# sehyun03/MulActSeg

Measured on AMD Instinct MI355X. Metric: superpixels scored/sec, higher is better.
Workload: dtype f32

## Files before the change

### include/mulactseg_hip.h

```cpp
#ifndef MULACTSEG_HIP_H
#define MULACTSEG_HIP_H

#include <stddef.h>
#include <stdint.h>

#ifdef __cplusplus
extern "C" {
#endif

#define MAS_ID_I64 0
#define MAS_ID_I32 1
#define MAS_ID_U16 2
#define MAS_MAP_U8 3

#define MAS_MAX_CLASSES 32

#define MAS_SCORE_FRAC_BITS 40
#define MAS_PROB_FRAC_BITS 23
#define MAS_LOSS_FRAC_BITS 32

#define MAS_ABI_VERSION 9
int mas_abi_version(void);
const char* mas_error_string(int code);

// ... 50 lines not shown
                                uint64_t* gmax , uint64_t* acc , void* stream);
int mas_partial_loss_bwd_lowres(const float* zq, int h, int w, const void* spx, int spx_dtype, const uint8_t* mask,
                                const uint32_t* bits, const uint64_t* gmax, const float* scale , int N, int C, int H, int W,
                                int S, float invT, int flags, int64_t* dzq_fix , void* stream);
#define MAS_GRAD_FRAC_BITS 44
int mas_fix_to_float(const int64_t* fix, int64_t n, int frac_bits, float* out, void* stream);

size_t mas_partial_loss_work_bytes(int N, int S, int C, int flags);
int mas_partial_loss_fwd_fused(const float* z, int h, int w, const void* spx, int spx_dtype, const uint8_t* mask, const uint8_t* targets,
                               int cols_stored, int cols_used, const uint32_t* bits, int N, int C, int H, int W, int S, float invT, int flags,
                               const float* weights, void* work, size_t work_bytes, float* losses, void* stream);
int mas_partial_loss_bwd_fused(const float* z, int h, int w, const void* spx, int spx_dtype, const uint8_t* mask, const uint32_t* bits,
                               const void* work, const float* grad, const float* weights, int N, int C, int H, int W, int S, float invT,
                               int flags, float* dz, int64_t* dzq_fix, void* stream);


int mas_region_keys(const float* score, const uint8_t* valid, const int32_t* img_rank, int64_t n_img, int S,
                    uint64_t* keys , void* stream);

size_t mas_select_workspace_bytes(int64_t n);

int mas_sort_keys_desc(const uint64_t* keys_in, int64_t n, uint64_t* keys_out, void* workspace, size_t ws_bytes,
                       void* stream);

int mas_budget_walk(const uint64_t* sorted_keys, int64_t n, const uint8_t* region_cost, const int32_t* img_of_rank,
                    int S, int64_t budget, int64_t max_out, int64_t* n_selected,
                    int32_t* sel_img, int32_t* sel_id, float* sel_score, void* workspace, size_t ws_bytes, void* stream);

int mas_region_reweight(float* score, const int32_t* dominant, int64_t n, int ban_class, const float* cls_w ,
                        void* stream);

int mas_dominant_hist(const int32_t* dominant, int64_t n, int C, uint64_t* counts , void* stream);

int mas_minmax_normalize(float* scores, int64_t n, uint32_t* scratch2, void* stream);


#define MAS_LABELS_BAD_VALUE 1

int mas_region_label_counts(const void* spx, int spx_dtype, const uint8_t* labels, int H, int W, int nseg, int num_classes, int trim_k,
                            int32_t* full , int32_t* trimmed , int32_t* status ,
                            void* stream);

int mas_region_multi_hot(const int32_t* full, const int32_t* trimmed, const uint8_t* listed, int nseg, int num_classes,
                         uint8_t* bits , int64_t* size , void* stream);

int mas_region_dominant(const int32_t* full, const uint8_t* listed, const int32_t* drawn , int nseg, int num_classes,
// ... 181 lines not shown
```

### mulactseg_amd/_lib.py

```python
import ctypes
import os

_HERE = os.path.dirname(os.path.abspath(__file__))
LIB_PATH = os.environ.get("MAS_LIB") or os.path.join(_HERE, "libmulactseg_hip.so")

ID_I64, ID_I32, ID_U16 = 0, 1, 2
MAP_U8 = 3
MAX_CLASSES = 32
LABELS_BAD_VALUE = 1
SCORE_FRAC, PROB_FRAC, LOSS_FRAC = 40, 23, 32
LOSS_CE, LOSS_GROUP, LOSS_GROUP_ONLY_MULTI, LOSS_DECOMP, LOSS_TCE = 1, 2, 4, 8, 16
ACC_WORDS = 8
GRAD_FRAC = 44
MS_MAX_SOURCES = 16

SK_DMA, SK_NOSPLIT = 1, 2
LOWRES_GENERIC = 1
ABI_VERSION = 9

_c = ctypes
_vp, _i, _f, _i64, _d = _c.c_void_p, _c.c_int, _c.c_float, _c.c_int64, _c.c_double


class SkOpts(ctypes.Structure):
    _fields_ = [("flags", _c.c_uint), ("spin_limit", _c.c_uint), ("stamps", _c.c_void_p)]


SIGNATURES = {
    "mas_abi_version": (_i, []),
    "mas_error_string": (_c.c_char_p, [_i]),
    "mas_class_prob_sum": (_i, [_vp, _i, _i, _i, _i, _f, _vp, _vp]),
    "mas_bvsb_region_accum": (_i, [_vp, _vp, _i, _vp, _i, _i, _i, _i, _i, _f, _vp, _vp, _vp]),
    "mas_region_finalize": (_i, [_vp, _vp, _i64, _i, _i, _vp, _vp, _vp, _vp, _vp]),
    "mas_region_keys": (_i, [_vp, _vp, _vp, _i64, _i, _vp, _vp]),
    "mas_select_workspace_bytes": (_c.c_size_t, [_i64]),
    "mas_sort_keys_desc": (_i, [_vp, _i64, _vp, _vp, _c.c_size_t, _vp]),
    "mas_budget_walk": (_i, [_vp, _i64, _vp, _vp, _i, _i64, _i64, _vp, _vp, _vp, _vp, _vp, _c.c_size_t, _vp]),
    "mas_region_reweight": (_i, [_vp, _vp, _i64, _i, _vp, _vp]),
    "mas_dominant_hist": (_i, [_vp, _i64, _i, _vp, _vp]),
    "mas_minmax_normalize": (_i, [_vp, _i64, _vp, _vp]),
    "mas_region_label_counts": (_i, [_vp, _i, _vp, _i, _i, _i, _i, _i, _vp, _vp, _vp, _vp]),
    "mas_region_multi_hot": (_i, [_vp, _vp, _vp, _i, _i, _vp, _vp, _vp]),
    "mas_region_dominant": (_i, [_vp, _vp, _vp, _i, _i, _i, _vp, _vp]),
    "mas_region_paint": (_i, [_vp, _i, _vp, _i, _i, _i, _vp, _i, _vp, _vp]),
    "mas_spx_max_onehot": (_i, [_vp, _i, _vp, _i, _i, _i, _i, _i, _vp, _vp, _vp, _vp, _vp]),
    "mas_iou_counts": (_i, [_vp, _vp, _vp, _i64, _i, _i64, _vp, _vp]),
    "mas_logits_iou_counts": (_i, [_vp, _vp, _i, _i, _i, _i, _i, _i64, _vp, _vp]),
    "mas_single_pass_accum": (_i, [_vp, _vp, _i, _i, _i, _i, _i, _i, _f, _vp, _vp, _vp, _vp]),
    "mas_single_pass_accum_lowres": (_i, [_vp, _i, _i, _vp, _i, _i, _i, _i, _i, _i, _f, _vp, _vp, _vp, _vp]),
    "mas_single_pass_accum_lowres_opt": (_i, [_vp, _i, _i, _vp, _i, _i, _i, _i, _i, _i, _f, _vp, _vp, _vp, _c.c_uint, _vp]),
    "mas_class_weight": (_i, [_vp, _i, _i, _i64, _i, _i, _d, _vp, _vp, _vp, _vp]),
    "mas_region_finalize_weighted": (_i, [_vp, _vp, _i64, _i, _vp, _i, _vp, _vp, _vp, _vp, _vp]),
    "mas_stage2_gather_protos": (_i, [_vp, _i, _i, _i, _i, _i, _vp, _i, _vp, _vp]),
    "mas_stage2_assign": (_i, [_vp, _i, _i, _i, _i, _i, _vp, _vp, _i, _vp, _vp, _vp, _vp, _vp]),
    "mas_stage2_adjacency": (_i, [_vp, _i, _i, _i, _vp, _vp, _vp]),
    "mas_stage2_propagate": (_i, [_vp, _i, _i, _i, _i, _i, _vp, _i, _vp, _vp, _vp, _vp, _vp, _vp, _vp, _vp]),
    "mas_aspp_dw3_fwd": (_i, [_vp, _vp, _vp, _vp, _i, _i, _i, _i, _i, _i, _i, _vp, _vp, _vp, _vp]),
    "mas_aspp_dw3_bwd_x": (_i, [_vp, _vp, _vp, _vp, _vp, _vp, _i, _i, _i, _i, _i, _i, _i, _vp, _vp]),
    "mas_aspp_dw3_bwd_w": (_i, [_vp, _vp, _vp, _vp, _i, _i, _i, _i, _i, _i, _i, _vp, _vp, _vp, _vp]),
# ... 128 lines not shown
```

### mulactseg_amd/active_selection/engine.py

```python
import numpy as np
import torch


class ShardPlan:

    def __init__(self, n_img, batch_size, rank=0, world=1):
        self.n_img, self.batch_size, self.rank, self.world = n_img, batch_size, rank, world
        self.n_batches = (n_img + batch_size - 1) // batch_size
        per = (self.n_batches + world - 1) // world
        self.batch_lo = min(rank * per, self.n_batches)
        self.batch_hi = min((rank + 1) * per, self.n_batches)
        self.img_lo = min(self.batch_lo * batch_size, n_img)
        self.img_hi = min(self.batch_hi * batch_size, n_img)
        self.per_rank_imgs = per * batch_size
        self.batch_of = (np.arange(n_img) // batch_size).astype(np.int32)

    @property
    def local_indices(self):
        return list(range(self.img_lo, self.img_hi))

    @property
    def n_local(self):
        return self.img_hi - self.img_lo

# ... 68 lines not shown
    def class_weight(self, prob_sum, hw, batch_size, n_batches, coeff):
        cum, w, w31 = self.ops.class_weight(prob_sum.contiguous(), hw, batch_size, n_batches, coeff)
        w._mas_w31 = w31
        return cum, w

    def finalize_weighted(self, class_sum, hist, cls_w, ban_class, want_hist_i64=False):
        w31 = None if cls_w is None else getattr(cls_w, '_mas_w31', None)
        if w31 is None:
            w = torch.ones(hist.shape[-1], dtype=torch.float32, device=hist.device) if cls_w is None else cls_w.detach().to(hist.device)
            w31 = (w.double() * 2147483648.0).floor().to(torch.int64).view(torch.int32)[::2].contiguous()
        return self.ops.region_finalize_weighted(class_sum, hist, w31, ban_class, want_hist_i64)

    def minmax_normalize_(self, scores):
        return self.ops.minmax_normalize_(scores)

    def region_reweight_(self, scores, dominant, ban_class, cls_w):
        return self.ops.region_reweight_(scores, dominant, ban_class, cls_w)

    def dominant_hist(self, dominant, C):
        return self.ops.dominant_hist(dominant, C)

    def select(self, scores, valid, img_rank, img_of_rank, region_cost, budget, max_out):
        keys = self.ops.region_keys(scores, valid, img_rank)
        skeys = self.ops.sort_keys_desc(keys)
        nsel, simg, sid, ssc = self.ops.budget_walk(skeys, region_cost, img_of_rank, scores.shape[1], budget, max_out)
        n = int(nsel.item())
        return n, simg[:n].cpu().numpy(), sid[:n].cpu().numpy(), ssc[:n].cpu().numpy()

    def local_head(self, plan, scores, valid, img_rank, max_out):
        lo, hi = plan.img_lo, plan.img_hi
        head = torch.zeros(max_out, dtype=torch.int64, device=scores.device)
        if hi > lo:
            keys = self.ops.region_keys(scores[lo:hi].contiguous(), None if valid is None else valid[lo:hi].contiguous(),
                                        img_rank[lo:hi].contiguous())
            m = min(keys.numel(), max_out)
            head[:m] = self.ops.sort_keys_desc(keys)[:m]
        return head

    def walk_heads(self, heads, region_cost, img_of_rank, S, budget, max_out):
        nsel, simg, sid, ssc = self.ops.budget_walk(self.ops.sort_keys_desc(heads), region_cost, img_of_rank, S, budget, max_out)
        n = int(nsel.item())
        return n, simg[:n].cpu().numpy(), sid[:n].cpu().numpy(), ssc[:n].cpu().numpy()

    def select_sharded(self, plan, scores, valid, img_rank, img_of_rank, region_cost, budget, max_out):
        head = self.local_head(plan, scores, valid, img_rank, max_out)
        merged = torch.empty(plan.world * max_out, dtype=torch.int64, device=scores.device)
        _dist().all_gather_into_tensor(merged, head)
        return self.walk_heads(merged, region_cost, img_of_rank, scores.shape[1], budget, max_out)


def default_backend(device):
    return HipBackend(device)


def select_regions(backend, plan, scores, valid, img_rank, img_of_rank, region_cost, budget, max_out):
    if plan.world > 1 and max_out is not None and _dist() is not None and hasattr(backend, 'select_sharded'):
        return backend.select_sharded(plan, scores, valid, img_rank, img_of_rank, region_cost, budget, max_out)
    return backend.select(scores, valid, img_rank, img_of_rank, region_cost, budget, max_out)


class AcquisitionRound:

    def __init__(self, n_img, n_channels, n_superpixels, batch_size, temperature, backend, rank=None, world=None,
                 single_pass=False):
        r, w = current_rank_world()
# ... 97 lines not shown
```

### mulactseg_amd/csrc/select.hip

```cpp
#include <cstring>

#include <rocprim/device/device_radix_sort.hpp>
#include <rocprim/device/device_scan.hpp>

#include "common.h"

namespace {

constexpr int kThreads = 256;

__device__ __forceinline__ unsigned order_bits(float f) {
    const unsigned b = mas_f2u(f);
    return (b & 0x80000000u) ? ~b : (b | 0x80000000u);
}
__device__ __forceinline__ float unorder_bits(unsigned o) {
    return mas_u2f((o & 0x80000000u) ? (o & 0x7fffffffu) : ~o);
}

inline int id_bits_for(int S) {
    int b = 1;
    while ((1LL << b) < S) ++b;
    return b;
}

// ... 102 lines not shown
    }
#pragma unroll
    for (int off = MAS_WAVE / 2; off > 0; off >>= 1) {
        const unsigned l2 = __shfl_down(lo, off, MAS_WAVE), h2 = __shfl_down(hi, off, MAS_WAVE);
        lo = l2 < lo ? l2 : lo;
        hi = h2 > hi ? h2 : hi;
    }
    if ((threadIdx.x & (MAS_WAVE - 1)) == 0) {
        atomicMin(&mm[0], lo);
        atomicMax(&mm[1], hi);
    }
}

__global__ void k_minmax_init(unsigned* mm) { mm[0] = 0xffffffffu; mm[1] = 0u; }

__global__ __launch_bounds__(kThreads) void k_minmax_apply(float* __restrict__ u, long long n, const unsigned* __restrict__ mm) {
    const long long i = (long long)blockIdx.x * kThreads + threadIdx.x;
    if (i >= n) return;
    const float mn = unorder_bits(mm[0]);
    const float mx = unorder_bits(mm[1]) - mn;
    u[i] = (u[i] - mn) / mx;
}

inline size_t align_up(size_t v) { return (v + 255) & ~(size_t)255; }

size_t sort_temp_bytes(long long n) {
    size_t bytes = 0;
    mas_u64* nul = nullptr;
    (void)rocprim::radix_sort_keys_desc(nullptr, bytes, nul, nul, (size_t)n, 0, 64, (hipStream_t)0);
    return bytes;
}
size_t scan_temp_bytes(long long n) {
    size_t bytes = 0;
    unsigned* nul = nullptr;
    (void)rocprim::inclusive_scan(nullptr, bytes, nul, nul, (size_t)n, rocprim::plus<unsigned>(), (hipStream_t)0);
    return bytes;
}

}

extern "C" size_t mas_select_workspace_bytes(int64_t n) {
    if (n <= 0) return 0;
    const size_t t = sort_temp_bytes(n), u = scan_temp_bytes(n);
    return align_up(t > u ? t : u) + 2 * align_up(sizeof(unsigned) * (size_t)n) + 256;
}

extern "C" int mas_region_keys(const float* score, const uint8_t* valid, const int32_t* img_rank, int64_t n_img, int S,
                               uint64_t* keys, void* stream) {
    if (!score || !img_rank || !keys) return MAS_ERR_NULL;
    if (n_img <= 0 || S <= 0) return MAS_ERR_SHAPE;
    const int b = id_bits_for(S);
    if (b > 24 || n_img > (1LL << (32 - b))) return MAS_ERR_RANGE;
    const long long n = (long long)n_img * S;
    const long long nblk = (n + kThreads - 1) / kThreads;
    if (nblk > 0x7fffffffLL) return MAS_ERR_SHAPE;
    hipLaunchKernelGGL(k_region_keys, dim3((unsigned)nblk), dim3(kThreads), 0, static_cast<hipStream_t>(stream), score, valid,
                       img_rank, n, S, b, reinterpret_cast<mas_u64*>(keys));
    return mas_launch_status();
}

extern "C" int mas_sort_keys_desc(const uint64_t* keys_in, int64_t n, uint64_t* keys_out, void* workspace, size_t ws_bytes,
                                  void* stream) {
    if (!keys_in || !keys_out || !workspace) return MAS_ERR_NULL;
    if (n <= 0) return MAS_ERR_SHAPE;
    size_t need = sort_temp_bytes(n);
    if (ws_bytes < need) return MAS_ERR_WORKSPACE;
    hipError_t e = rocprim::radix_sort_keys_desc(workspace, need, reinterpret_cast<const mas_u64*>(keys_in),
                                                 reinterpret_cast<mas_u64*>(keys_out), (size_t)n, 0, 64,
                                                 static_cast<hipStream_t>(stream));
    return e == hipSuccess ? mas_launch_status() : (int)e;
}

extern "C" int mas_budget_walk(const uint64_t* sorted_keys, int64_t n, const uint8_t* region_cost, const int32_t* img_of_rank,
                               int S, int64_t budget, int64_t max_out, int64_t* n_selected, int32_t* sel_img, int32_t* sel_id,
                               float* sel_score, void* workspace, size_t ws_bytes, void* stream) {
    if (!sorted_keys || !img_of_rank || !n_selected || !sel_img || !sel_id || !sel_score || !workspace) return MAS_ERR_NULL;
    if (n <= 0 || S <= 0 || max_out <= 0 || budget < 0) return MAS_ERR_SHAPE;
    if (n > (1LL << 24)) return MAS_ERR_RANGE;
    if (ws_bytes < mas_select_workspace_bytes(n)) return MAS_ERR_WORKSPACE;
    hipStream_t st = static_cast<hipStream_t>(stream);
    const int b = id_bits_for(S);
    unsigned char* ws = static_cast<unsigned char*>(workspace);
    size_t temp = scan_temp_bytes(n);
    const size_t t = sort_temp_bytes(n);
    const size_t temp_region = align_up(t > temp ? t : temp);
    unsigned* cost = reinterpret_cast<unsigned*>(ws + temp_region);
    unsigned* prefix = reinterpret_cast<unsigned*>(ws + temp_region + align_up(sizeof(unsigned) * (size_t)n));
    const mas_u64* keys = reinterpret_cast<const mas_u64*>(sorted_keys);
    unsigned long long* nsel = reinterpret_cast<unsigned long long*>(n_selected);
    const long long nblk = (n + kThreads - 1) / kThreads;
    hipLaunchKernelGGL(k_set_u64, dim3(1), dim3(1), 0, st, nsel, (unsigned long long)n);
    hipLaunchKernelGGL(k_walk_cost, dim3((unsigned)nblk), dim3(kThreads), 0, st, keys, (long long)n, region_cost, img_of_rank, S, b, cost);
// ... 41 lines not shown
```

### mulactseg_amd/csrc/single_pass.hip

```cpp
#include <cstdlib>
#include "common.h"

namespace {

constexpr int kThreads = 256;
constexpr int kTileW = 256;
constexpr int kTileH = 16;
constexpr int kLogSlots = 7;
constexpr int kSlots = 1 << kLogSlots;

__device__ __forceinline__ int table_slot(int* keys, int id) {
    unsigned h = ((unsigned)id * 2654435769u) >> (32 - kLogSlots);
    for (int probe = 0; probe < kSlots; ++probe) {
        int k = __hip_atomic_load(&keys[h], __ATOMIC_RELAXED, __HIP_MEMORY_SCOPE_WORKGROUP);
        if (k == id) return (int)h;
        if (k == -1) {
            int old = atomicCAS(&keys[h], -1, id);
            if (old == -1 || old == id) return (int)h;
        }
        h = (h + 1) & (kSlots - 1);
    }
    return -1;
}

// ... 284 lines not shown
    __device__ __forceinline__ void load(const unsigned short* p) { a = *reinterpret_cast<const uint2*>(p); }
    __device__ __forceinline__ void get(int (&id)[4]) const {
        id[0] = (int)(a.x & 0xffffu); id[1] = (int)(a.x >> 16); id[2] = (int)(a.y & 0xffffu); id[3] = (int)(a.y >> 16);
    }
};

template <int CT, typename IdT>
struct RowRegs {
    float4 t[CT];
    IdQuad<IdT> ids;
};

template <int CT, bool EXACT, typename IdT>
__device__ __forceinline__ void ring_issue(RowRegs<CT, IdT>& r, const float* __restrict__ zb, const IdT* __restrict__ sb, int C,
                                           int HW, unsigned off) {
    r.ids.load(sb + off);
#pragma unroll
    for (int c = 0; c < CT; ++c) {
        if (EXACT || c < C) r.t[c] = mas_load_stream4(zb + (size_t)c * HW + off);
        else r.t[c] = make_float4(0.f, 0.f, 0.f, 0.f);
    }
}

template <int CT, bool EXACT, typename IdT>
__device__ __forceinline__ void ring_consume(RowRegs<CT, IdT>& r, bool ok, int C, int S, float invT, unsigned* s_acc, int* t_keys,
                                             mas_u64* t_sum, unsigned* t_hist, mas_u64* __restrict__ gsum,
                                             unsigned* __restrict__ ghist, int& last_id, int& last_slot) {
    mas_v2f v[2][CT];
    float b1[4], b2[4];
    int a1[4];
#pragma unroll
    for (int k = 0; k < 4; ++k) { b1[k] = -__builtin_inff(); b2[k] = -__builtin_inff(); a1[k] = 0; }
#pragma unroll
    for (int c = 0; c < CT; ++c) {
        if (EXACT || c < C) {
            const float4 t = r.t[c];
            v[0][c] = (mas_v2f){t.x, t.y};
            v[1][c] = (mas_v2f){t.z, t.w};
            const float q[4] = {t.x, t.y, t.z, t.w};
#pragma unroll
            for (int k = 0; k < 4; ++k) {
                const bool g1 = q[k] > b1[k];
                b2[k] = __builtin_amdgcn_fmed3f(b1[k], b2[k], q[k]);
                a1[k] = g1 ? c : a1[k];
                b1[k] = __builtin_amdgcn_fmed3f(b1[k], q[k], 3.402823466e+38f);
            }
        } else {
            v[0][c] = mas_splat(0.f);
            v[1][c] = mas_splat(0.f);
        }
    }
    __builtin_amdgcn_sched_barrier(0);
    {
        mas_v2f Ra, Rb;
        mas_softmax_quad<CT, EXACT, true>(v[0], v[1], C, invT, Ra, Rb, (mas_v2f){b1[0], b1[1]}, (mas_v2f){b1[2], b1[3]});
        Ra = Ra * mas_splat(8388608.0f);
        Rb = Rb * mas_splat(8388608.0f);
        Ra = ok ? Ra : mas_splat(0.0f);
        Rb = ok ? Rb : mas_splat(0.0f);
#pragma unroll
        for (int c = 0; c < CT; ++c) {
            if (EXACT || c < C) {
                const mas_v2f ta = mas_pk_fma(v[0][c], Ra, mas_splat(8388608.0f));
                const mas_v2f tb = mas_pk_fma(v[1][c], Rb, mas_splat(8388608.0f));
                lds_add(&s_acc[c * kThreads + threadIdx.x], (mas_f2u(ta.x) + mas_f2u(ta.y)) + (mas_f2u(tb.x) + mas_f2u(tb.y)));
            }
        }
    }
    __builtin_amdgcn_sched_barrier(0);
    mas_u64 q[4];
    int key[4], id[4];
    float margin[4];
    r.ids.get(id);
    mas_bvsb_quad(b1, b2, invT, margin);
#pragma unroll
    for (int k = 0; k < 4; ++k) {
        id[k] = (ok && id[k] >= 0 && id[k] < S) ? id[k] : -1;
        q[k] = mas_fix_unit(margin[k]);
        key[k] = id[k] < 0 ? -1 : id[k] * MAS_MAX_CLASSES + a1[k];
    }
    const bool same = (key[0] == key[1]) && (key[1] == key[2]) && (key[2] == key[3]);
    if (same) {
        if (key[0] >= 0) {
            if (id[0] != last_id) {
                last_slot = table_slot(t_keys, id[0]);
                last_id = id[0];
            }
            const int s = last_slot;
            const mas_u64 qs = (q[0] + q[1]) + (q[2] + q[3]);
            if (s >= 0) {
                lds_add(&t_sum[s * C + a1[0]], qs);
                lds_add(&t_hist[s * C + a1[0]], 4u);
            } else {
                atomicAdd(&gsum[(size_t)id[0] * C + a1[0]], qs);
                atomicAdd(&ghist[(size_t)id[0] * C + a1[0]], 4u);
            }
        }
    } else {
#pragma unroll
        for (int k = 0; k < 4; ++k) {
            if (key[k] < 0) continue;
            const int s = table_slot(t_keys, id[k]);
            if (s >= 0) {
                lds_add(&t_sum[s * C + a1[k]], q[k]);
                lds_add(&t_hist[s * C + a1[k]], 1u);
            } else {
                atomicAdd(&gsum[(size_t)id[k] * C + a1[k]], q[k]);
                atomicAdd(&ghist[(size_t)id[k] * C + a1[k]], 1u);
            }
        }
    }
}

template <int CT, bool EXACT, typename IdT>
__global__ __launch_bounds__(kThreads, 2) void k_single_pass_ring(const float* __restrict__ z, const IdT* __restrict__ spx, int C,
                                                                   int H, int W, int S, float invT, int tiles_x, int tiles_y,
                                                                   mas_u64* __restrict__ prob_sum,
                                                                   mas_u64* __restrict__ class_sum, unsigned* __restrict__ hist) {
    extern __shared__ __attribute__((aligned(16))) unsigned char smem[];
    mas_u64* t_sum = reinterpret_cast<mas_u64*>(smem);
    mas_u64* s_part = reinterpret_cast<mas_u64*>(smem + sizeof(mas_u64) * kSlots * C);
    unsigned* t_hist = reinterpret_cast<unsigned*>(smem + sizeof(mas_u64) * (kSlots * C + 4 * CT));
    int* t_keys = reinterpret_cast<int*>(smem + sizeof(mas_u64) * (kSlots * C + 4 * CT) + sizeof(unsigned) * kSlots * C);
    unsigned* s_acc = reinterpret_cast<unsigned*>(t_keys + kSlots);

    for (int i = threadIdx.x; i < kSlots; i += kThreads) t_keys[i] = -1;
    for (int i = threadIdx.x; i < kSlots * C; i += kThreads) { t_sum[i] = 0; t_hist[i] = 0; }
#pragma unroll
    for (int c = 0; c < CT; ++c) s_acc[c * kThreads + threadIdx.x] = 0;
    __syncthreads();

    int bid = blockIdx.x;
    const int tx = bid % tiles_x; bid /= tiles_x;
    const int ty = bid % tiles_y;
    const int b = bid / tiles_y;
    const int HW = H * W;
    const float* zb = z + (size_t)b * C * HW;
    const IdT* sb = spx + (size_t)b * HW;
    mas_u64* gsum = class_sum + (size_t)b * S * C;
    unsigned* ghist = hist + (size_t)b * S * C;
    const int lane = threadIdx.x & (MAS_WAVE - 1);
    const int wave = threadIdx.x / MAS_WAVE;

    const int x0 = tx * kTileW + lane * 4;
    const bool okx = x0 < W;
    const unsigned xc = okx ? (unsigned)x0 : 0u;
    const int ybase = ty * kRingTileH + wave;
    auto off_of = [&](int it) -> unsigned {
        int y = ybase + it * 4;
        y = y < H ? y : H - 1;
        return (unsigned)y * (unsigned)W + xc;
    };
    auto ok_of = [&](int it) -> bool { return okx && (ybase + it * 4 < H); };

    RowRegs<CT, IdT> A, B;
    int last_id = -2, last_slot = -1;
    ring_issue<CT, EXACT, IdT>(A, zb, sb, C, HW, off_of(0));
#pragma unroll 1
    for (int it = 0; it < kRingRows; it += 2) {
        ring_issue<CT, EXACT, IdT>(B, zb, sb, C, HW, off_of(it + 1));
        __builtin_amdgcn_sched_barrier(0);
        ring_consume<CT, EXACT, IdT>(A, ok_of(it), C, S, invT, s_acc, t_keys, t_sum, t_hist, gsum, ghist, last_id, last_slot);
        __builtin_amdgcn_sched_barrier(0);
        ring_issue<CT, EXACT, IdT>(A, zb, sb, C, HW, off_of(it + 2 < kRingRows ? it + 2 : kRingRows - 1));
        __builtin_amdgcn_sched_barrier(0);
        ring_consume<CT, EXACT, IdT>(B, ok_of(it + 1), C, S, invT, s_acc, t_keys, t_sum, t_hist, gsum, ghist, last_id, last_slot);
        __builtin_amdgcn_sched_barrier(0);
    }

    __syncthreads();
#pragma unroll
    for (int c = 0; c < CT; ++c) {
        mas_u64 a = s_acc[c * kThreads + threadIdx.x] - (unsigned)(kRingRows * 4) * MAS_PROBQ_BIAS;
#pragma unroll
        for (int off = MAS_WAVE / 2; off > 0; off >>= 1) a += __shfl_down(a, off, MAS_WAVE);
        if (lane == 0) s_part[wave * CT + c] = a;
    }
    __syncthreads();
    if (threadIdx.x < CT && (EXACT || (int)threadIdx.x < C)) {
        mas_u64 a = 0;
#pragma unroll
        for (int w = 0; w < kThreads / MAS_WAVE; ++w) a += s_part[w * CT + threadIdx.x];
        if (a) atomicAdd(&prob_sum[(size_t)b * C + threadIdx.x], a);
    }
    for (int i = threadIdx.x; i < kSlots * C; i += kThreads) {
        const unsigned n = t_hist[i];
        if (n) {
            const int s = i / C;
            const size_t g = (size_t)t_keys[s] * C + (i - s * C);
            atomicAdd(&ghist[g], n);
// ... 25 lines not shown
    __syncthreads();
    if ((long long)threadIdx.x >= rows) return;
    const long long r = r0 + threadIdx.x;
    const unsigned* h = s_hist + threadIdx.x * CP;
    const mas_u64* cs = s_sum + threadIdx.x * CP;
    unsigned long long n = 0;
    unsigned best = 0;
    int arg = 0;
    uint64_t hi = 0, lo = 0;
    for (int c = 0; c < C; ++c) {
        const unsigned v = h[c];
        n += v;
        if (v > best) { best = v; arg = c; }
        if (v) mas_mac_u64_u32((uint64_t)cs[c], w31[c], &hi, &lo);
    }
    float sc = 0.0f;
    if (n) sc = mas_fixed_mean(mas_shr31_u128(hi, lo), n, MAS_SCORE_FRAC);
    if (ban_class >= 0 && arg == ban_class) sc = 0.0f;
    score[r] = sc;
    if (dominant) dominant[r] = arg;
    if (count) count[r] = (unsigned)n;
}

inline bool mas_ring_enabled() {
    static const bool on = [] { const char* e = getenv("MAS_SINGLE_PASS_RING"); return !(e && e[0] == '0'); }();
    return on;
}

inline size_t smem_bytes(int C, int CT) {
    return sizeof(mas_u64) * ((size_t)kSlots * C + 4 * CT) + sizeof(unsigned) * (size_t)kSlots * C + sizeof(int) * kSlots;
}

template <int CT, bool EXACT, typename IdT>
int launch(const float* z, const void* spx, int B, int C, int H, int W, int S, float invT, mas_u64* prob_sum, mas_u64* class_sum,
           unsigned* hist, hipStream_t st) {
    const int tiles_x = (W + kTileW - 1) / kTileW;
    const int tiles_y = (H + kTileH - 1) / kTileH;
    const long long nblk = (long long)B * tiles_x * tiles_y;
    if (nblk <= 0 || nblk > 0x7fffffffLL) return MAS_ERR_SHAPE;
    const bool vec = (W % 4 == 0) && (((uintptr_t)z & 15) == 0);
    const size_t smem = smem_bytes(C, CT);
    const IdT* ids = static_cast<const IdT*>(spx);
    if constexpr (EXACT) if (vec && H >= kRingTileH && (((uintptr_t)spx & 15) == 0) && mas_ring_enabled()) {
        const int rtiles_y = (H + kRingTileH - 1) / kRingTileH;
        const long long rblk = (long long)B * tiles_x * rtiles_y;
        hipLaunchKernelGGL((k_single_pass_ring<CT, EXACT, IdT>), dim3((unsigned)rblk), dim3(kThreads),
                           smem + sizeof(unsigned) * CT * kThreads, st, z, ids, C, H, W, S, invT, tiles_x, rtiles_y, prob_sum,
                           class_sum, hist);
        return mas_launch_status();
    }
    if (vec)
        hipLaunchKernelGGL((k_single_pass<CT, EXACT, IdT, true>), dim3((unsigned)nblk), dim3(kThreads), smem, st, z, ids, C, H, W, S,
                           invT, tiles_x, tiles_y, prob_sum, class_sum, hist);
    else
        hipLaunchKernelGGL((k_single_pass<CT, EXACT, IdT, false>), dim3((unsigned)nblk), dim3(kThreads), smem, st, z, ids, C, H, W, S,
                           invT, tiles_x, tiles_y, prob_sum, class_sum, hist);
    return mas_launch_status();
}

template <int CT, bool EXACT, typename IdT>
int launch_low(const float* zq, int h, int w, const void* spx, int B, int C, int H, int W, int S, float invT, mas_u64* prob_sum,
               mas_u64* class_sum, unsigned* hist, unsigned flags, hipStream_t st) {
    const int tiles_x = (W + kTileW - 1) / kTileW;
    const int tiles_y = (H + kTileH - 1) / kTileH;
    const long long nblk = (long long)B * tiles_x * tiles_y;
    if (nblk <= 0 || nblk > 0x7fffffffLL) return MAS_ERR_SHAPE;
    const LowSrc lr{h, w, (float)h / (float)H, (float)w / (float)W};
    if ((double)kTileH * h / H + 2.0 > kLowRows || (double)kTileW * w / W + 2.0 > kLowCols) return MAS_ERR_RANGE;
    const size_t smem = smem_bytes(C, CT) + sizeof(float) * (size_t)C * kLowRows * kLowCols;
    const bool vec = (W % 4 == 0);
    const IdT* ids = static_cast<const IdT*>(spx);
// ... 111 lines not shown
```

### mulactseg_amd/ops.py

```python
import ctypes
import os

import numpy as np
import torch

from . import _lib

_ID_CODES = {torch.int64: _lib.ID_I64, torch.int32: _lib.ID_I32, torch.uint16: _lib.ID_U16,
             torch.int16: _lib.ID_U16}


def inv_temperature(T):
    return float(np.float32(1.0) / np.float32(T))


def _stream(t):
    return torch.cuda.current_stream(t.device).cuda_stream


def _need(t, name, dtype=None):
    if not t.is_cuda:
        raise _lib.MulActSegHipError("%s must live on the GPU (no CPU path exists)" % name)
    if dtype is not None and t.dtype != dtype:
        raise TypeError("%s must be %s, got %s" % (name, dtype, t.dtype))
# ... 266 lines not shown
        valid = _mask_u8(valid)
        if tuple(valid.shape) != (n_img, S):
            raise ValueError("valid must be [n_img, S]")
    keys = torch.empty(n_img * S, dtype=torch.int64, device=scores.device)
    with torch.cuda.device(scores.device):
        _lib.check(_lib.load().mas_region_keys(scores.data_ptr(), valid.data_ptr() if valid is not None else None,
                                               img_rank.data_ptr(), n_img, S, keys.data_ptr(), _stream(scores)),
                   "mas_region_keys")
    return keys


def sort_keys_desc(keys):
    _need(keys, "keys", torch.int64)
    n = keys.numel()
    lib = _lib.load()
    ws = torch.empty(lib.mas_select_workspace_bytes(n), dtype=torch.uint8, device=keys.device)
    out = torch.empty_like(keys)
    with torch.cuda.device(keys.device):
        _lib.check(lib.mas_sort_keys_desc(keys.data_ptr(), n, out.data_ptr(), ws.data_ptr(), ws.numel(), _stream(keys)),
                   "mas_sort_keys_desc")
    return out


def budget_walk(sorted_keys, region_cost, img_of_rank, S, budget, max_out=None):
    _need(sorted_keys, "sorted_keys", torch.int64)
    _need(img_of_rank, "img_of_rank", torch.int32)
    cost_bits = region_cost
    if cost_bits is not None:
        _need(cost_bits, "region_cost", torch.uint8)
    n = sorted_keys.numel()
    max_out = n if max_out is None else min(n, max_out)
    dev = sorted_keys.device
    lib = _lib.load()
    ws = torch.empty(lib.mas_select_workspace_bytes(n), dtype=torch.uint8, device=dev)
    nsel = torch.empty(1, dtype=torch.int64, device=dev)
    sel_img = torch.empty(max_out, dtype=torch.int32, device=dev)
    sel_id = torch.empty(max_out, dtype=torch.int32, device=dev)
    sel_score = torch.empty(max_out, dtype=torch.float32, device=dev)
    with torch.cuda.device(dev):
        _lib.check(lib.mas_budget_walk(sorted_keys.data_ptr(), n, cost_bits.data_ptr() if cost_bits is not None else None,
                                       img_of_rank.data_ptr(), S, int(budget), max_out, nsel.data_ptr(), sel_img.data_ptr(),
                                       sel_id.data_ptr(), sel_score.data_ptr(), ws.data_ptr(), ws.numel(), _stream(sorted_keys)),
                   "mas_budget_walk")
    return nsel, sel_img, sel_id, sel_score


def minmax_normalize_(scores):
    _need(scores, "scores", torch.float32)
    scratch = torch.empty(2, dtype=torch.int32, device=scores.device)
    with torch.cuda.device(scores.device):
        _lib.check(_lib.load().mas_minmax_normalize(scores.data_ptr(), scores.numel(), scratch.data_ptr(), _stream(scores)),
                   "mas_minmax_normalize")
    return scores


def iou_counts(outputs, outputs_all, targets, num_classes, ignore_label, counts=None):
    _need(targets, "targets", torch.int64)
    if outputs is not None:
        _need(outputs, "outputs", torch.int64)
    if outputs_all is not None:
        _need(outputs_all, "outputs_all", torch.int64)
    if counts is None:
        counts = torch.zeros(3 * num_classes + 3, dtype=torch.int64, device=targets.device)
    with torch.cuda.device(targets.device):
        _lib.check(_lib.load().mas_iou_counts(outputs.data_ptr() if outputs is not None else None,
                                              outputs_all.data_ptr() if outputs_all is not None else None,
                                              targets.data_ptr(), targets.numel(), num_classes, int(ignore_label),
# ... 1704 lines not shown
```

Before: 56.45 million.

## Replace full key sort with radix top-k selection and batch walk results into one copy

```diff
diff --git a/include/mulactseg_hip.h b/include/mulactseg_hip.h
--- a/include/mulactseg_hip.h
+++ b/include/mulactseg_hip.h
@@ -96,6 +96,9 @@
 
 int mas_sort_keys_desc(const uint64_t* keys_in, int64_t n, uint64_t* keys_out, void* workspace, size_t ws_bytes,
                        void* stream);
+
+int mas_select_top(const uint64_t* keys, int64_t n, int64_t k, uint64_t* top , void* workspace, size_t ws_bytes,
+                   void* stream);
 
 int mas_budget_walk(const uint64_t* sorted_keys, int64_t n, const uint8_t* region_cost, const int32_t* img_of_rank,
                     int S, int64_t budget, int64_t max_out, int64_t* n_selected,
diff --git a/mulactseg_amd/_lib.py b/mulactseg_amd/_lib.py
--- a/mulactseg_amd/_lib.py
+++ b/mulactseg_amd/_lib.py
@@ -35,6 +35,7 @@
     "mas_region_keys": (_i, [_vp, _vp, _vp, _i64, _i, _vp, _vp]),
     "mas_select_workspace_bytes": (_c.c_size_t, [_i64]),
     "mas_sort_keys_desc": (_i, [_vp, _i64, _vp, _vp, _c.c_size_t, _vp]),
+    "mas_select_top": (_i, [_vp, _i64, _i64, _vp, _vp, _c.c_size_t, _vp]),
     "mas_budget_walk": (_i, [_vp, _i64, _vp, _vp, _i, _i64, _i64, _vp, _vp, _vp, _vp, _vp, _c.c_size_t, _vp]),
     "mas_region_reweight": (_i, [_vp, _vp, _i64, _i, _vp, _vp]),
     "mas_dominant_hist": (_i, [_vp, _i64, _i, _vp, _vp]),
diff --git a/mulactseg_amd/active_selection/engine.py b/mulactseg_amd/active_selection/engine.py
--- a/mulactseg_amd/active_selection/engine.py
+++ b/mulactseg_amd/active_selection/engine.py
@@ -114,10 +114,17 @@
 
     def select(self, scores, valid, img_rank, img_of_rank, region_cost, budget, max_out):
         keys = self.ops.region_keys(scores, valid, img_rank)
-        skeys = self.ops.sort_keys_desc(keys)
-        nsel, simg, sid, ssc = self.ops.budget_walk(skeys, region_cost, img_of_rank, scores.shape[1], budget, max_out)
-        n = int(nsel.item())
-        return n, simg[:n].cpu().numpy(), sid[:n].cpu().numpy(), ssc[:n].cpu().numpy()
+        return self._order_and_walk(keys, region_cost, img_of_rank, scores.shape[1], budget, max_out)
+
+    def _order_and_walk(self, keys, region_cost, img_of_rank, S, budget, max_out):
+        n_keys = keys.numel()
+        if max_out is not None:
+            k = max_out + 1
+            if k < n_keys and (k <= self.ops.SELECT_TOP_LDS_KEYS or 8 * k <= n_keys):
+                res = self.ops.budget_walk_host(self.ops.select_top(keys, k), region_cost, img_of_rank, S, budget, max_out)
+                if res[0] <= max_out:
+                    return res
+        return self.ops.budget_walk_host(self.ops.sort_keys_desc(keys), region_cost, img_of_rank, S, budget, max_out)
 
     def local_head(self, plan, scores, valid, img_rank, max_out):
         lo, hi = plan.img_lo, plan.img_hi
@@ -130,9 +137,7 @@
         return head
 
     def walk_heads(self, heads, region_cost, img_of_rank, S, budget, max_out):
-        nsel, simg, sid, ssc = self.ops.budget_walk(self.ops.sort_keys_desc(heads), region_cost, img_of_rank, S, budget, max_out)
-        n = int(nsel.item())
-        return n, simg[:n].cpu().numpy(), sid[:n].cpu().numpy(), ssc[:n].cpu().numpy()
+        return self._order_and_walk(heads, region_cost, img_of_rank, S, budget, max_out)
 
     def select_sharded(self, plan, scores, valid, img_rank, img_of_rank, region_cost, budget, max_out):
         head = self.local_head(plan, scores, valid, img_rank, max_out)
diff --git a/mulactseg_amd/csrc/select.hip b/mulactseg_amd/csrc/select.hip
--- a/mulactseg_amd/csrc/select.hip
+++ b/mulactseg_amd/csrc/select.hip
@@ -148,6 +148,137 @@
     u[i] = (u[i] - mn) / mx;
 }
 
+constexpr int kSelBits = 11;
+constexpr int kSelBins = 1 << kSelBits;
+constexpr int kSelPasses = (64 + kSelBits - 1) / kSelBits;
+constexpr int kSelLdsKeys = 8192;
+constexpr int kSelGrid = 1024;
+constexpr int kSelKeysPerThread = 4;
+
+struct SelState {
+    mas_u64 prefix;
+    unsigned long long need;
+    unsigned long long taken;
+};
+
+__device__ __forceinline__ int sel_shift(int d) { const int s = 64 - kSelBits * (d + 1); return s > 0 ? s : 0; }
+__device__ __forceinline__ int sel_width(int d) { return 64 - kSelBits * d - sel_shift(d); }
+
+__device__ void sel_resolve(const unsigned* __restrict__ hist_prev, const SelState* __restrict__ st_prev, int d_prev, SelState& out) {
+    constexpr int kPer = kSelBins / kThreads;
+    constexpr int kWaves = kThreads / MAS_WAVE;
+    __shared__ unsigned long long s_wave[kWaves];
+    __shared__ SelState s_out;
+    const int t = threadIdx.x, lane = t & (MAS_WAVE - 1), wave = t / MAS_WAVE;
+    const int hi = kSelBins - t * kPer;
+    unsigned c[kPer];
+    unsigned long long mine = 0;
+#pragma unroll
+    for (int j = 0; j < kPer; ++j) { c[j] = hist_prev[hi - 1 - j]; mine += c[j]; }
+    unsigned long long incl = mine;
+#pragma unroll
+    for (int off = 1; off < MAS_WAVE; off <<= 1) {
+        const unsigned long long y = __shfl_up(incl, off, MAS_WAVE);
+        if (lane >= off) incl += y;
+    }
+    if (lane == MAS_WAVE - 1) s_wave[wave] = incl;
+    const SelState p = *st_prev;
+    __syncthreads();
+    unsigned long long above = incl - mine;
+    for (int w = 0; w < wave; ++w) above += s_wave[w];
+    if (above < p.need && p.need <= above + mine) {
+        int j = 0;
+        while (j < kPer - 1 && above + c[j] < p.need) above += c[j++];
+        s_out.prefix = p.prefix | ((mas_u64)(hi - 1 - j) << sel_shift(d_prev));
+        s_out.need = p.need - above;
+        s_out.taken = 0;
+    }
+    __syncthreads();
+    out = s_out;
+}
+
+__global__ __launch_bounds__(kThreads) void k_sel_hist(const mas_u64* __restrict__ keys, long long n, long long k, int d,
+                                                       unsigned* __restrict__ hist, SelState* __restrict__ st) {
+    __shared__ unsigned s_h[kSelBins];
+    SelState cur{0ull, (unsigned long long)k, 0ull};
+    if (d > 0) sel_resolve(hist + (size_t)(d - 1) * kSelBins, st + (d - 1), d - 1, cur);
+    if (blockIdx.x == 0 && threadIdx.x == 0) st[d] = cur;
+    for (int i = threadIdx.x; i < kSelBins; i += kThreads) s_h[i] = 0;
+    __syncthreads();
+    const int sh = sel_shift(d);
+    const int hi_shift = sh + sel_width(d);
+    const mas_u64 hmask = hi_shift >= 64 ? 0ull : (~0ull << hi_shift);
+    const unsigned dmask = (1u << sel_width(d)) - 1u;
+    for (long long b0 = (long long)blockIdx.x * kThreads * kSelKeysPerThread; b0 < n; b0 += (long long)gridDim.x * kThreads * kSelKeysPerThread) {
+        mas_u64 kv[kSelKeysPerThread];
+#pragma unroll
+        for (int j = 0; j < kSelKeysPerThread; ++j) {
+            const long long i = b0 + j * kThreads + threadIdx.x;
+            kv[j] = i < n ? keys[i] : 0ull;
+        }
+#pragma unroll
+        for (int j = 0; j < kSelKeysPerThread; ++j) {
+            const long long i = b0 + j * kThreads + threadIdx.x;
+            if (i < n && (kv[j] & hmask) == cur.prefix) atomicAdd(&s_h[(unsigned)(kv[j] >> sh) & dmask], 1u);
+        }
+    }
+    __syncthreads();
+    unsigned* h = hist + (size_t)d * kSelBins;
+    for (int i = threadIdx.x; i < kSelBins; i += kThreads)
+        if (s_h[i]) atomicAdd(&h[i], s_h[i]);
+}
+
+__global__ __launch_bounds__(kThreads) void k_sel_compact(const mas_u64* __restrict__ keys, long long n, long long k,
+                                                          const unsigned* __restrict__ hist, SelState* __restrict__ st,
+                                                          mas_u64* __restrict__ out) {
+    SelState fin;
+    sel_resolve(hist + (size_t)(kSelPasses - 1) * kSelBins, st + (kSelPasses - 1), kSelPasses - 1, fin);
+    const mas_u64 T = fin.prefix;
+    const long long n_gt = k - (long long)fin.need;
+    unsigned long long* taken = &st[kSelPasses].taken;
+    const int lane = threadIdx.x & (MAS_WAVE - 1);
+    const long long stride = (long long)gridDim.x * kThreads;
+    for (long long b0 = (long long)blockIdx.x * kThreads * kSelKeysPerThread; b0 < n; b0 += stride * kSelKeysPerThread) {
+        mas_u64 kv[kSelKeysPerThread];
+#pragma unroll
+        for (int j = 0; j < kSelKeysPerThread; ++j) {
+            const long long i = b0 + j * kThreads + threadIdx.x;
+            kv[j] = i < n ? keys[i] : 0ull;
+        }
+#pragma unroll
+        for (int j = 0; j < kSelKeysPerThread; ++j) {
+            const bool take = b0 + j * kThreads + threadIdx.x < n && kv[j] > T;
+            const unsigned long long m = __ballot(take);
+            if (!m) continue;
+            unsigned long long base = 0;
+            if (lane == 0) base = atomicAdd(taken, (unsigned long long)__popcll(m));
+            base = __shfl(base, 0, MAS_WAVE);
+            const unsigned long long at = base + __popcll(m & ((1ull << lane) - 1ull));
+            if (take && at < (unsigned long long)n_gt) out[at] = kv[j];
+        }
+    }
+    for (long long i = n_gt + (long long)blockIdx.x * kThreads + threadIdx.x; i < k; i += stride) out[i] = T;
+}
+
+constexpr int kSelRankSplit = 16;
+__global__ __launch_bounds__(kThreads) void k_sel_rank_sort(const mas_u64* __restrict__ keys, int k, mas_u64* __restrict__ out) {
+    __shared__ mas_u64 s[kSelLdsKeys];
+    for (int i = threadIdx.x; i < k; i += kThreads) s[i] = keys[i];
+    __syncthreads();
+    const int i = blockIdx.x * (kThreads / kSelRankSplit) + threadIdx.x / kSelRankSplit;
+    const int part = threadIdx.x % kSelRankSplit;
+    const mas_u64 me = i < k ? s[i] : 0ull;
+    unsigned r = 0;
+#pragma unroll 8
+    for (int j = part; j < k; j += kSelRankSplit) {
+        const mas_u64 o = s[j];
+        r += (o > me) || (o == me && j < i);
+    }
+#pragma unroll
+    for (int off = 1; off < kSelRankSplit; off <<= 1) r += __shfl_xor(r, off, MAS_WAVE);
+    if (i < k && part == 0 && r < (unsigned)k) out[r] = me;
+}
+
 inline size_t align_up(size_t v) { return (v + 255) & ~(size_t)255; }
 
 size_t sort_temp_bytes(long long n) {
@@ -163,12 +294,21 @@
     return bytes;
 }
 
+size_t top_bytes(long long k) {
+    size_t b = align_up(sizeof(unsigned) * kSelBins * kSelPasses) + align_up(sizeof(SelState) * (kSelPasses + 1));
+    b += align_up(sizeof(mas_u64) * (size_t)k);
+    if (k > kSelLdsKeys) b += align_up(sort_temp_bytes(k));
+    return b;
+}
+
 }
 
 extern "C" size_t mas_select_workspace_bytes(int64_t n) {
     if (n <= 0) return 0;
     const size_t t = sort_temp_bytes(n), u = scan_temp_bytes(n);
-    return align_up(t > u ? t : u) + 2 * align_up(sizeof(unsigned) * (size_t)n) + 256;
+    const size_t walk = align_up(t > u ? t : u) + 2 * align_up(sizeof(unsigned) * (size_t)n) + 256;
+    const size_t top = top_bytes(n);
+    return walk > top ? walk : top;
 }
 
 extern "C" int mas_region_keys(const float* score, const uint8_t* valid, const int32_t* img_rank, int64_t n_img, int S,
@@ -194,6 +334,37 @@
     hipError_t e = rocprim::radix_sort_keys_desc(workspace, need, reinterpret_cast<const mas_u64*>(keys_in),
                                                  reinterpret_cast<mas_u64*>(keys_out), (size_t)n, 0, 64,
                                                  static_cast<hipStream_t>(stream));
+    return e == hipSuccess ? mas_launch_status() : (int)e;
+}
+
+extern "C" int mas_select_top(const uint64_t* keys, int64_t n, int64_t k, uint64_t* top, void* workspace, size_t ws_bytes, void* stream) {
+    if (!keys || !top || !workspace) return MAS_ERR_NULL;
+    if (n <= 0 || k <= 0 || k > n) return MAS_ERR_SHAPE;
+    if (ws_bytes < top_bytes(k)) return MAS_ERR_WORKSPACE;
+    hipStream_t st = static_cast<hipStream_t>(stream);
+    unsigned char* ws = static_cast<unsigned char*>(workspace);
+    const size_t hist_bytes = align_up(sizeof(unsigned) * kSelBins * kSelPasses);
+    const size_t state_bytes = align_up(sizeof(SelState) * (kSelPasses + 1));
+    unsigned* hist = reinterpret_cast<unsigned*>(ws);
+    SelState* state = reinterpret_cast<SelState*>(ws + hist_bytes);
+    const mas_u64* in = reinterpret_cast<const mas_u64*>(keys);
+    mas_u64* out = reinterpret_cast<mas_u64*>(top);
+    hipError_t e = hipMemsetAsync(ws, 0, hist_bytes + state_bytes, st);
+    if (e != hipSuccess) return (int)e;
+    long long nblk = (n + kThreads * kSelKeysPerThread - 1) / (kThreads * kSelKeysPerThread);
+    if (nblk > kSelGrid) nblk = kSelGrid;
+    for (int d = 0; d < kSelPasses; ++d)
+        hipLaunchKernelGGL(k_sel_hist, dim3((unsigned)nblk), dim3(kThreads), 0, st, in, (long long)n, (long long)k, d, hist, state);
+    mas_u64* dst = reinterpret_cast<mas_u64*>(ws + hist_bytes + state_bytes);
+    hipLaunchKernelGGL(k_sel_compact, dim3((unsigned)nblk), dim3(kThreads), 0, st, in, (long long)n, (long long)k, hist, state, dst);
+    if (k <= kSelLdsKeys) {
+        const int per = kThreads / kSelRankSplit;
+        hipLaunchKernelGGL(k_sel_rank_sort, dim3((unsigned)((k + per - 1) / per)), dim3(kThreads), 0, st, dst, (int)k, out);
+        return mas_launch_status();
+    }
+    size_t need = sort_temp_bytes(k);
+    void* tmp = ws + hist_bytes + state_bytes + align_up(sizeof(mas_u64) * (size_t)k);
+    e = rocprim::radix_sort_keys_desc(tmp, need, dst, out, (size_t)k, 0, 64, st);
     return e == hipSuccess ? mas_launch_status() : (int)e;
 }
 
diff --git a/mulactseg_amd/csrc/single_pass.hip b/mulactseg_amd/csrc/single_pass.hip
--- a/mulactseg_amd/csrc/single_pass.hip
+++ b/mulactseg_amd/csrc/single_pass.hip
@@ -1,4 +1,5 @@
 #include <cstdlib>
+#include <cstring>
 #include "common.h"
 
 namespace {
@@ -330,10 +331,12 @@
     }
 }
 
-template <int CT, bool EXACT, typename IdT>
+template <int CT, bool EXACT, typename IdT, bool REFILL = false>
 __device__ __forceinline__ void ring_consume(RowRegs<CT, IdT>& r, bool ok, int C, int S, float invT, unsigned* s_acc, int* t_keys,
                                              mas_u64* t_sum, unsigned* t_hist, mas_u64* __restrict__ gsum,
-                                             unsigned* __restrict__ ghist, int& last_id, int& last_slot) {
+                                             unsigned* __restrict__ ghist, int& last_id, int& last_slot,
+                                             const float* __restrict__ zb = nullptr, const IdT* __restrict__ sb = nullptr,
+                                             int HW = 0, unsigned off_next = 0u) {
     mas_v2f v[2][CT];
     float b1[4], b2[4];
     int a1[4];
@@ -359,6 +362,12 @@
         }
     }
     __builtin_amdgcn_sched_barrier(0);
+    int id[4];
+    if (REFILL) {
+        r.ids.get(id);
+        r.ids.load(sb + off_next);
+        __builtin_amdgcn_sched_barrier(0);
+    }
     {
         mas_v2f Ra, Rb;
         mas_softmax_quad<CT, EXACT, true>(v[0], v[1], C, invT, Ra, Rb, (mas_v2f){b1[0], b1[1]}, (mas_v2f){b1[2], b1[3]});
@@ -372,14 +381,20 @@
                 const mas_v2f ta = mas_pk_fma(v[0][c], Ra, mas_splat(8388608.0f));
                 const mas_v2f tb = mas_pk_fma(v[1][c], Rb, mas_splat(8388608.0f));
                 lds_add(&s_acc[c * kThreads + threadIdx.x], (mas_f2u(ta.x) + mas_f2u(ta.y)) + (mas_f2u(tb.x) + mas_f2u(tb.y)));
+                if (REFILL) {
+                    r.t[c] = mas_load_stream4(zb + (size_t)c * HW + off_next);
+                    __builtin_amdgcn_sched_barrier(0);
+                }
+            } else if (REFILL) {
+                r.t[c] = make_float4(0.f, 0.f, 0.f, 0.f);
             }
         }
     }
     __builtin_amdgcn_sched_barrier(0);
     mas_u64 q[4];
-    int key[4], id[4];
+    int key[4];
     float margin[4];
-    r.ids.get(id);
+    if (!REFILL) r.ids.get(id);
     mas_bvsb_quad(b1, b2, invT, margin);
 #pragma unroll
     for (int k = 0; k < 4; ++k) {
@@ -420,7 +435,7 @@
     }
 }
 
-template <int CT, bool EXACT, typename IdT>
+template <int CT, bool EXACT, typename IdT, bool CLASS_REFILL>
 __global__ __launch_bounds__(kThreads, 2) void k_single_pass_ring(const float* __restrict__ z, const IdT* __restrict__ spx, int C,
                                                                    int H, int W, int S, float invT, int tiles_x, int tiles_y,
                                                                    mas_u64* __restrict__ prob_sum,
@@ -464,16 +479,34 @@
     RowRegs<CT, IdT> A, B;
     int last_id = -2, last_slot = -1;
     ring_issue<CT, EXACT, IdT>(A, zb, sb, C, HW, off_of(0));
+    if constexpr (CLASS_REFILL) {
+        __builtin_amdgcn_sched_barrier(0);
+        ring_issue<CT, EXACT, IdT>(B, zb, sb, C, HW, off_of(1));
 #pragma unroll 1
-    for (int it = 0; it < kRingRows; it += 2) {
-        ring_issue<CT, EXACT, IdT>(B, zb, sb, C, HW, off_of(it + 1));
+        for (int it = 0; it < kRingRows - 2; it += 2) {
+            __builtin_amdgcn_sched_barrier(0);
+            ring_consume<CT, EXACT, IdT, true>(A, ok_of(it), C, S, invT, s_acc, t_keys, t_sum, t_hist, gsum, ghist, last_id, last_slot,
+                                               zb, sb, HW, off_of(it + 2));
+            __builtin_amdgcn_sched_barrier(0);
+            ring_consume<CT, EXACT, IdT, true>(B, ok_of(it + 1), C, S, invT, s_acc, t_keys, t_sum, t_hist, gsum, ghist, last_id,
+                                               last_slot, zb, sb, HW, off_of(it + 3));
+        }
         __builtin_amdgcn_sched_barrier(0);
-        ring_consume<CT, EXACT, IdT>(A, ok_of(it), C, S, invT, s_acc, t_keys, t_sum, t_hist, gsum, ghist, last_id, last_slot);
+        ring_consume<CT, EXACT, IdT>(A, ok_of(kRingRows - 2), C, S, invT, s_acc, t_keys, t_sum, t_hist, gsum, ghist, last_id, last_slot);
         __builtin_amdgcn_sched_barrier(0);
-        ring_issue<CT, EXACT, IdT>(A, zb, sb, C, HW, off_of(it + 2 < kRingRows ? it + 2 : kRingRows - 1));
-        __builtin_amdgcn_sched_barrier(0);
-        ring_consume<CT, EXACT, IdT>(B, ok_of(it + 1), C, S, invT, s_acc, t_keys, t_sum, t_hist, gsum, ghist, last_id, last_slot);
-        __builtin_amdgcn_sched_barrier(0);
+        ring_consume<CT, EXACT, IdT>(B, ok_of(kRingRows - 1), C, S, invT, s_acc, t_keys, t_sum, t_hist, gsum, ghist, last_id, last_slot);
+    } else {
+#pragma unroll 1
+        for (int it = 0; it < kRingRows; it += 2) {
+            ring_issue<CT, EXACT, IdT>(B, zb, sb, C, HW, off_of(it + 1));
+            __builtin_amdgcn_sched_barrier(0);
+            ring_consume<CT, EXACT, IdT>(A, ok_of(it), C, S, invT, s_acc, t_keys, t_sum, t_hist, gsum, ghist, last_id, last_slot);
+            __builtin_amdgcn_sched_barrier(0);
+            ring_issue<CT, EXACT, IdT>(A, zb, sb, C, HW, off_of(it + 2 < kRingRows ? it + 2 : kRingRows - 1));
+            __builtin_amdgcn_sched_barrier(0);
+            ring_consume<CT, EXACT, IdT>(B, ok_of(it + 1), C, S, invT, s_acc, t_keys, t_sum, t_hist, gsum, ghist, last_id, last_slot);
+            __builtin_amdgcn_sched_barrier(0);
+        }
     }
 
     __syncthreads();
@@ -545,9 +578,15 @@
     if (count) count[r] = (unsigned)n;
 }
 
-inline bool mas_ring_enabled() {
-    static const bool on = [] { const char* e = getenv("MAS_SINGLE_PASS_RING"); return !(e && e[0] == '0'); }();
-    return on;
+enum RingForm { kRingOff, kRingRow, kRingClass };
+inline RingForm mas_ring_form() {
+    static const RingForm f = [] {
+        const char* e = getenv("MAS_SINGLE_PASS_RING");
+        if (e && e[0] == '0') return kRingOff;
+        if (e && strcmp(e, "class") == 0) return kRingClass;
+        return kRingRow;
+    }();
+    return f;
 }
 
 inline size_t smem_bytes(int C, int CT) {
@@ -564,12 +603,17 @@
     const bool vec = (W % 4 == 0) && (((uintptr_t)z & 15) == 0);
     const size_t smem = smem_bytes(C, CT);
     const IdT* ids = static_cast<const IdT*>(spx);
-    if constexpr (EXACT) if (vec && H >= kRingTileH && (((uintptr_t)spx & 15) == 0) && mas_ring_enabled()) {
+    if constexpr (EXACT) if (vec && H >= kRingTileH && (((uintptr_t)spx & 15) == 0) && mas_ring_form() != kRingOff) {
         const int rtiles_y = (H + kRingTileH - 1) / kRingTileH;
         const long long rblk = (long long)B * tiles_x * rtiles_y;
-        hipLaunchKernelGGL((k_single_pass_ring<CT, EXACT, IdT>), dim3((unsigned)rblk), dim3(kThreads),
-                           smem + sizeof(unsigned) * CT * kThreads, st, z, ids, C, H, W, S, invT, tiles_x, rtiles_y, prob_sum,
-                           class_sum, hist);
+        if (mas_ring_form() != kRingClass)
+            hipLaunchKernelGGL((k_single_pass_ring<CT, EXACT, IdT, false>), dim3((unsigned)rblk), dim3(kThreads),
+                               smem + sizeof(unsigned) * CT * kThreads, st, z, ids, C, H, W, S, invT, tiles_x, rtiles_y, prob_sum,
+                               class_sum, hist);
+        else
+            hipLaunchKernelGGL((k_single_pass_ring<CT, EXACT, IdT, true>), dim3((unsigned)rblk), dim3(kThreads),
+                               smem + sizeof(unsigned) * CT * kThreads, st, z, ids, C, H, W, S, invT, tiles_x, rtiles_y, prob_sum,
+                               class_sum, hist);
         return mas_launch_status();
     }
     if (vec)
diff --git a/mulactseg_amd/ops.py b/mulactseg_amd/ops.py
--- a/mulactseg_amd/ops.py
+++ b/mulactseg_amd/ops.py
@@ -312,7 +312,36 @@
     return out
 
 
+SELECT_TOP_LDS_KEYS = 8192
+
+
+def select_top(keys, k):
+    _need(keys, "keys", torch.int64)
+    n = keys.numel()
+    if not 0 < k <= n:
+        raise ValueError("select_top needs 0 < k <= keys.numel(), got k=%d of %d" % (k, n))
+    lib = _lib.load()
+    ws = torch.empty(lib.mas_select_workspace_bytes(n), dtype=torch.uint8, device=keys.device)
+    out = torch.empty(k, dtype=torch.int64, device=keys.device)
+    with torch.cuda.device(keys.device):
+        _lib.check(lib.mas_select_top(keys.data_ptr(), n, k, out.data_ptr(), ws.data_ptr(), ws.numel(), _stream(keys)), "mas_select_top")
+    return out
+
+
 def budget_walk(sorted_keys, region_cost, img_of_rank, S, budget, max_out=None):
+    return _budget_walk(sorted_keys, region_cost, img_of_rank, S, budget, max_out)[1:]
+
+
+def budget_walk_host(sorted_keys, region_cost, img_of_rank, S, budget, max_out=None):
+    buf, _, _, _, _ = _budget_walk(sorted_keys, region_cost, img_of_rank, S, budget, max_out)
+    h = buf.cpu().numpy()
+    m = (h.size - 8) // 12
+    n = int(h[:8].view(np.int64)[0])
+    return (n, h[8:8 + 4 * m].view(np.int32)[:n], h[8 + 4 * m:8 + 8 * m].view(np.int32)[:n],
+            h[8 + 8 * m:8 + 12 * m].view(np.float32)[:n])
+
+
+def _budget_walk(sorted_keys, region_cost, img_of_rank, S, budget, max_out):
     _need(sorted_keys, "sorted_keys", torch.int64)
     _need(img_of_rank, "img_of_rank", torch.int32)
     cost_bits = region_cost
@@ -323,16 +352,17 @@
     dev = sorted_keys.device
     lib = _lib.load()
     ws = torch.empty(lib.mas_select_workspace_bytes(n), dtype=torch.uint8, device=dev)
-    nsel = torch.empty(1, dtype=torch.int64, device=dev)
-    sel_img = torch.empty(max_out, dtype=torch.int32, device=dev)
-    sel_id = torch.empty(max_out, dtype=torch.int32, device=dev)
-    sel_score = torch.empty(max_out, dtype=torch.float32, device=dev)
+    buf = torch.empty(8 + 12 * max_out, dtype=torch.uint8, device=dev)
+    nsel = buf[:8].view(torch.int64)
+    sel_img = buf[8:8 + 4 * max_out].view(torch.int32)
+    sel_id = buf[8 + 4 * max_out:8 + 8 * max_out].view(torch.int32)
+    sel_score = buf[8 + 8 * max_out:].view(torch.float32)
     with torch.cuda.device(dev):
         _lib.check(lib.mas_budget_walk(sorted_keys.data_ptr(), n, cost_bits.data_ptr() if cost_bits is not None else None,
                                        img_of_rank.data_ptr(), S, int(budget), max_out, nsel.data_ptr(), sel_img.data_ptr(),
                                        sel_id.data_ptr(), sel_score.data_ptr(), ws.data_ptr(), ws.numel(), _stream(sorted_keys)),
                    "mas_budget_walk")
-    return nsel, sel_img, sel_id, sel_score
+    return buf, nsel, sel_img, sel_id, sel_score
 
 
 def minmax_normalize_(scores):
```

Result: no change. 56.72 million, median of 6 (+0.5%).
